# BosonHBC/BHRayTracer

Hardware: AMD Instinct MI355X
Metric: Mrays/s (closest-hit + any-hit rays per second), with wall-clock per frame (higher is better)
Workload: dtype f32

## Files before the change

### bhraytracer_amd/__init__.py

```python
import ctypes as C
import os

import numpy as np

from .flat import FlatView

_HERE = os.path.dirname(os.path.abspath(__file__))
LIB_PATH = os.environ.get("BHRT_LIB") or os.path.join(_HERE, "libbhrt.so")

SIDE_FRONT, SIDE_BACK, SIDE_BOTH = 1, 2, 3


class BhrtError(RuntimeError):
    pass


class Info(C.Structure):
    _fields_ = [("width", C.c_int32), ("height", C.c_int32)] + [
        (n, C.c_uint32) for n in ("n_nodes", "n_meshes", "n_triangles", "n_bvh_nodes", "n_materials", "n_lights",
                                  "n_textures", "max_node_depth", "max_bvh_depth")] + [
        ("flat_bytes", C.c_uint64), ("n_warnings", C.c_uint32)]


class Opts(C.Structure):
    _fields_ = [("spp", C.c_int32), ("gi_bounces", C.c_int32), ("internal_bounces", C.c_int32), ("seed", C.c_uint32),
                ("jitter", C.c_int32), ("gamma", C.c_int32), ("photon_map", C.c_int32),
                ("rank", C.c_int32), ("world_size", C.c_int32), ("tile_size", C.c_int32),
                ("samples_per_pass", C.c_int32), ("timers", C.c_int32), ("photon_exact", C.c_int32), ("leaf_skip", C.c_int32), ("photon_radius", C.c_float), ("lens", C.c_int32)]


class Stats(C.Structure):
    _fields_ = [("closest_rays", C.c_uint64), ("shadow_rays", C.c_uint64), ("shade_calls", C.c_uint64),
                ("camera_samples", C.c_uint64), ("passes", C.c_uint32), ("wave_iterations", C.c_uint32),
                ("seconds_total", C.c_double), ("seconds_trace_closest", C.c_double),
                ("seconds_trace_shadow", C.c_double), ("seconds_shade", C.c_double), ("seconds_other", C.c_double),
                ("launches_trace_closest", C.c_uint64), ("launches_trace_shadow", C.c_uint64),
                ("seconds_photon_gather", C.c_double), ("seconds_photon_heavy", C.c_double),
                ("photon_queries", C.c_uint64), ("photon_heavy_queries", C.c_uint64), ("photon_wave_queries", C.c_uint64),
                ("photon_exact_queries", C.c_uint64), ("photon_nodes_visited", C.c_uint64), ("deferred_rays", C.c_uint64),
                ("photon_lane_queries", C.c_uint64), ("photon_lane_nodes", C.c_uint64), ("photon_found", C.c_uint64), ("reserved", C.c_double * 1)]

    def as_dict(self):
        return {n: getattr(self, n) for n, _ in self._fields_ if n != "reserved"}


class DenoiseOpts(C.Structure):
    _fields_ = [("iterations", C.c_int32), ("sigma_normal", C.c_float), ("sigma_depth", C.c_float), ("sigma_luminance", C.c_float),
                ("gamma", C.c_int32), ("reserved", C.c_int32 * 3)]


class AdaptiveOpts(C.Structure):
    _fields_ = [("min_spp", C.c_int32), ("threshold", C.c_float), ("floor", C.c_float), ("reserved", C.c_int32 * 5)]


class Hits(C.Structure):
    _fields_ = [("t", C.c_void_p), ("node", C.c_void_p), ("prim", C.c_void_p), ("front", C.c_void_p)]


_lib = None

EXPORTS = [
    "bhrt_last_error", "bhrt_default_opts", "bhrt_scene_load_xml", "bhrt_scene_free", "bhrt_scene_info",
    "bhrt_scene_warning", "bhrt_scene_flat", "bhrt_scene_upload", "bhrt_device_count",
# ... 362 lines not shown
```

### bhraytracer_amd/csrc/device_color24.h

```cpp
#pragma once
#include <stddef.h>
#include <stdint.h>

#include "bhrt_detmath.h"
#include "vecmath.h"

namespace bhrt {

__device__ inline void store_color24(uint8_t *rgb8, size_t pix, V3 out, int gamma)
{
    if (gamma) {
        const float inv = 1 / 2.2f;
        out = v3(dm::powf_(out.x, inv), dm::powf_(out.y, inv), dm::powf_(out.z, inv));
    }
    int r = int(out.x * 255 + 0.5f), g = int(out.y * 255 + 0.5f), b = int(out.z * 255 + 0.5f);
    rgb8[pix * 3] = (uint8_t)(r < 0 ? 0 : (r > 255 ? 255 : r));
    rgb8[pix * 3 + 1] = (uint8_t)(g < 0 ? 0 : (g > 255 ? 255 : g));
    rgb8[pix * 3 + 2] = (uint8_t)(b < 0 ? 0 : (b > 255 ? 255 : b));
}

}
```

### bhraytracer_amd/csrc/device_state.h

```cpp
#pragma once

namespace bhrt {

template <class T> struct DevBuf {
    T *p = nullptr;
    size_t n = 0;
    DevBuf() = default;
    DevBuf(const DevBuf &) = delete;
    DevBuf &operator=(const DevBuf &) = delete;
    DevBuf(DevBuf &&o) noexcept : p(o.p), n(o.n) { o.p = nullptr; o.n = 0; }
    DevBuf &operator=(DevBuf &&o) noexcept
    {
        if (this != &o) { Free(); p = o.p; n = o.n; o.p = nullptr; o.n = 0; }
        return *this;
    }
    ~DevBuf() { Free(); }
    int Reserve(size_t want)
    {
        if (n >= want) return BHRT_OK;
        Free();
        HIP_CHECK(hipMalloc(&p, want * sizeof(T)));
        n = want;
        return BHRT_OK;
    }
// ... 49 lines not shown
        if (stream2) (void)hipStreamDestroy(stream2);
        if (stream) (void)hipStreamDestroy(stream);
    }
};

struct DeviceState : DeviceQueues {
    int device = -1;
    uint32_t n_cus = 256;
    DevBuf<uint8_t> d_blob;
    DevBuf<int32_t> d_chain;
    DevBuf<float> d_aux;
    DevScene S;
    uint32_t cap_samples = 0, cap_rays = 0, cap_frames = 0;
    DevBuf<float> d_rayf[2];
    DevBuf<uint32_t> d_rayu[2];
    DevBuf<float> d_hitf;
    DevBuf<int32_t> d_hiti;
    DevBuf<float> d_shf;
    DevBuf<uint32_t> d_shu;
    DevBuf<uint32_t> d_fu;
    DevBuf<uint64_t> d_fcode;
    DevBuf<float> d_ff;
    DevBuf<float> d_samples;
    DevBuf<uint32_t> d_order;
    uint32_t order_shard_cap = 0;
    DevBuf<uint32_t> d_seg;
    DevBuf<uint32_t> d_park;
    DevBuf<float> d_slowf;
    DevBuf<uint32_t> d_slowu;
    DevBuf<float> d_shf2;
    DevBuf<uint32_t> d_shu2;
    DevBuf<uint32_t> d_order_sh;
    DevBuf<uint32_t> d_seg_sh;
    DevBuf<Counters> d_cnt_sh;
    DevBuf<Counters> d_cnt;
    PinnedBuf<HostCounters> h_pub;
    HostCounters *d_pub = nullptr;
    uint32_t pub_seq = 0;
    int timers = 0;
    int photon_exact = 0;
    uint32_t *d_knn = nullptr;
    DevBuf<uint32_t> d_sel;
    struct PendingTimer { int e0, e1; double *acc; };
    std::vector<PendingTimer> ev_pending;
    std::vector<int> ev_free;
    DevBuf<DPhoton> d_photons;
// ... 3 lines not shown
    DevBuf<float4> d_ph_hot, d_ph_cold, d_ph_dbox;
    PhotonMapDev pm;
    DevBuf<unsigned long long> d_scr;
    uint32_t scr_lanes = 0;
    uint32_t heavy_cap = 0;
    DevBuf<uint32_t> d_heavy;
    DevBuf<uint32_t> d_long;
    DevBuf<uint32_t> d_cell_of, d_gorder, d_rank_of, d_keys_out;
    DevBuf<uint8_t> d_sort_temp;
    size_t sort_temp_bytes = 0;
    DevBuf<uint32_t> d_n_heavy;
    PinnedBuf<uint32_t> h_n_heavy;
    DevBuf<uint32_t> d_cells, d_tile_sums;
    struct Knobs {
        int stream_waves = -1;
        bool fused_camera = true;
        bool no_slow_queue = false;
        bool debug_slow = false, debug_gather = false, debug_drain = false;
        bool balance_host = false;
        int frame_cap = 0;
        int gather_lane_budget = 0;
        bool gather_counting_sort = false;
        bool shadow_overlap = true;
        int gather_stats = 0;
        void FromEnv()
        {
            if (const char *e = getenv("BHRT_STREAM_WAVES")) stream_waves = atoi(e);
            if (const char *e = getenv("BHRT_FUSED_CAMERA")) fused_camera = atoi(e) != 0;
            no_slow_queue = getenv("BHRT_NO_SLOW_QUEUE") != nullptr;
            debug_slow = getenv("BHRT_DEBUG_SLOW") != nullptr; debug_gather = getenv("BHRT_DEBUG_GATHER") != nullptr; debug_drain = getenv("BHRT_DEBUG_DRAIN") != nullptr;
            if (const char *e = getenv("BHRT_PHOTON_BALANCE_HOST")) balance_host = atoi(e) != 0;
            if (const char *e = getenv("BHRT_GATHER_COUNTING_SORT")) gather_counting_sort = atoi(e) != 0;
            if (const char *e = getenv("BHRT_SHADOW_OVERLAP")) shadow_overlap = atoi(e) != 0;
        }
    } knobs;
    uint64_t pass_hint_key = 0;
    uint32_t pass_hint = 0;
    uint64_t frames_seen_key = 0;
    double frames_seen = 0;
    size_t frame_px = 0;
    DevBuf<uint8_t> d_frame_rgb;
    DevBuf<float> d_frame_rad, d_frame_var;
    DevBuf<uint32_t> d_frame_cnt;
    DevBuf<uint8_t> d_ad;
    DevBuf<uint8_t> d_dn;
    size_t api_cap = 0;
    DevBuf<float> d_api_f;
    DevBuf<int32_t> d_api_i;
};

void DestroyDeviceState(DeviceState *d)
{
    if (!d) return;
    if (d->device >= 0) (void)hipSetDevice(d->device);
    delete d;
}
// ... 3 lines not shown
```

### bhraytracer_amd/csrc/kernels.hip

```cpp
#include <hip/hip_runtime.h>

#include <stdlib.h>
#include <string.h>

#include <algorithm>
#include <type_traits>
#include <chrono>
#include <string>
#include <vector>

#include "bhrt.h"
#include "denoise.h"
#include "device_color24.h"
#include "device_photon.h"
#include "photon_host.h"
#include "scene_internal.h"

namespace bhrt {

#define HIP_CHECK(expr)                                                                                        \
    do {                                                                                                       \
        hipError_t e_ = (expr);                                                                                \
        if (e_ != hipSuccess) {                                                                                \
            SetError(std::string(#expr) + ": " + hipGetErrorString(e_));                                       \
// ... 100 lines not shown
    __syncthreads();
    if (threadIdx.x < 3) {
        const uint32_t k = threadIdx.x;
        uint32_t sum = 0;
        for (int w = 0; w < kShadeWaves; w++) { const uint32_t t = L.total[k][w]; L.base[k][w] = sum; sum += t; }
        uint32_t *ctr = k == 0 ? c0 : (k == 1 ? c1 : c2);
        const uint32_t b = (sum && ctr) ? atomicAdd(ctr, sum) : 0u;
        for (int w = 0; w < kShadeWaves; w++) L.base[k][w] += b;
    }
    __syncthreads();
    s0a = L.base[0][wave] + pa;
    s0b = L.base[0][wave] + ta + pb;
    s1 = L.base[1][wave] + (uint32_t)__popcll(m1 & lt);
    s2 = L.base[2][wave] + (uint32_t)__popcll(m2 & lt);
    __syncthreads();
}

__device__ inline uint32_t sample_addr(const PassInfo &P, uint32_t slot)
{
    uint32_t px, smp;
    fdivmod(slot, P.by_spp, px, smp);
    return smp * P.n_pixels + px;
}

__device__ inline void put_ray(const RayQueue &q, uint32_t i, V3 o, V3 d, uint32_t frame, uint32_t meta, uint32_t ctr)
{
    q.ox[i] = o.x; q.oy[i] = o.y; q.oz[i] = o.z; q.dx[i] = d.x; q.dy[i] = d.y; q.dz[i] = d.z;
    q.frame[i] = frame; q.meta[i] = meta;
    if ((meta & 15u) != RK_GI) q.rng_ctr[i] = ctr;
}
__device__ inline uint32_t make_meta(uint32_t kind, uint32_t side, int bounce) { return kind | (side << 4) | ((uint32_t)(bounce & 0xff) << 8); }
__device__ inline void st3(float *a, uint32_t i, V3 v) { a[3 * (size_t)i] = v.x; a[3 * (size_t)i + 1] = v.y; a[3 * (size_t)i + 2] = v.z; }
__device__ inline V3 ld3i(const float *a, uint32_t i) { return v3(a[3 * (size_t)i], a[3 * (size_t)i + 1], a[3 * (size_t)i + 2]); }

template <bool kLens = false>
__device__ inline bool camera_ray(const DevScene &S, const PassInfo &P, uint32_t idx, V3 &o, V3 &d)
{
    int i = 0, j = 0;
    uint32_t s;
    o = v3(0, 0, 0); d = v3(0, 0, 0);
    if (!slot_pixel(P, idx, i, j, s)) return false;
    const V3 topLeft = ld3(S.cam.top_left), ddx = ld3(S.cam.dd_x), ddy = ld3(S.cam.dd_y), pos = ld3(S.cam.pos);
    V3 target = (topLeft + (float)i * ddx) - (float)j * ddy;
    if (P.jitter) {
        const float pixelLen = P.pixel_len;
        const V3 ux = ld3(P.jx), uy = ld3(P.jy);
// ... 606 lines not shown
                    out.has_shadow = true;
                    out.so = a.p;
                    out.sd = light.size > 0 ? sample_along_normal(g, centerDir, light.size) : centerDir;
                    out.stmax = 1;
                }
            }
            const V3 kd = kd_s, ks = ks_s;
            st3(F.brdf, f, kd * cosTheta + ks * dm::powf_(dot(vH, vN), m.glossiness));
        }
    }
    if (R.photon) {
        st3(F.ph_p, f, a.p); st3(F.ph_n, f, a.N); st3(F.ph_v, f, vV);
        st3(F.ph_kd, f, kd_s);
        st3(F.ph_ks, f, ks_s);
    }
    F.info[f] = how | (dmode << 3) | (light_idx << 8) | (flags << 16) | ((uint32_t)(mi & 0xfff) << 20);
}

#ifndef BHRT_SHADE_WAVES
#define BHRT_SHADE_WAVES 4
#endif
template <bool kCamera, bool kTex, bool kFused = false>
__device__ __forceinline__ void shade_block(const DevScene &S, const RenderParams &R, const PassInfo &P, const RayQueue &qin, const HitBuf &hb, uint32_t n, const RayQueue &qout,
                                            const ShadowQueue &qs, const Frames &F, float *samples, Counters *cnt, const RayOrder &ord)
{
    static_assert(!kFused || kCamera, "only camera rays are traced in the shading kernel");
    __shared__ BlockAllocLds lds;
    uint32_t seg = 0, local = 0, i;
    bool active;
    if (kFused) {
        i = blockIdx.x * kShadeBlock + threadIdx.x;
        active = i < n;
        if (!active) i = 0;
    } else {
        constexpr uint32_t kSegs = 3 * BHRT_ORDER_SHARDS;
        __shared__ uint32_t s_seg;
        if (threadIdx.x < 64) {
            const uint32_t l = threadIdx.x;
            const uint32_t a = ord.seg_start[l], b = (l + 64 < kSegs) ? ord.seg_start[l + 64] : 0xffffffffu;
            const uint32_t n_le = (uint32_t)__popcll(__ballot(a <= blockIdx.x)) + (uint32_t)__popcll(__ballot(b <= blockIdx.x));
            if (l == 0) s_seg = n_le - 1;
        }
        __syncthreads();
        seg = s_seg;
        if (blockIdx.x >= ord.seg_start[kSegs]) return;
        const uint32_t seg_cnt = ord.seg_count[seg];
        const uint32_t bb = blockIdx.x - ord.seg_start[seg];
// ... 28 lines not shown
    uint32_t f, u2;
    if (kFused) { uint32_t u0, u1; block_alloc3(lds, &cnt->n_frames.v, new_frame ? 1u : 0u, 0u, nullptr, 0u, nullptr, 0u, f, u0, u1, u2); }
    else f = ord.frame_base[seg] + local;
    if (new_frame && f >= R.cap_frames) { flag_overflow(cnt, 1u); new_frame = false; }

    ShadeOut so;
    so.has_refr = so.has_gi = so.has_shadow = false;
    uint32_t ray_owner = owner;

    if (new_frame) {
        uint64_t code = 1;
        uint32_t skey;
        int gi;
        uint32_t how;
        V3 mult = v3(1, 1, 1);
        if (kind == RK_CAMERA) {
            int pi, pj;
            uint32_t osmp;
            slot_pixel(P, owner, pi, pj, osmp);
            skey = bhrt_sample_key(P.seed, (uint32_t)(pj * P.W + pi), P.s0 + osmp);
            gi = R.gi_bounces;
            bounce = R.internal_bounces;
            how = FH_ROOT;
        } else {
            const uint64_t pcode = F.code[owner];
            skey = F.skey[owner];
            const uint32_t pi2 = F.info2[owner];
            gi = (int)(pi2 & 0xffu) - 64 - 1;
            if (kind == RK_GI) {
                code = pcode * 2 + 1;
                how = FH_GI;
                bounce = (int)((pi2 >> 8) & 0xffu);
            } else if (kind == RK_REFR_IN) {
                code = pcode * 2;
                how = FH_REFR_FRONT;
            } else {
                code = pcode * 2;
                how = FH_REFR_OUT;
                const bhrt_material &pm = S.materials[(F.info[owner] >> 20) & 0xfffu];
                V3 af = v3(dm::powf_(BHRT_EULER, -pm.absorption[0] * hit.t), dm::powf_(BHRT_EULER, -pm.absorption[1] * hit.t),
                           dm::powf_(BHRT_EULER, -pm.absorption[2] * hit.t));
                mult = ld3i(F.refr_color, owner) * af;
            }
        }
        F.parent[f] = owner;
        F.info2[f] = (uint32_t)(gi + 64) | ((uint32_t)(bounce & 0xff) << 8);
        F.skey[f] = skey;
        F.code[f] = code;
        if (how == FH_REFR_OUT) st3(F.mult, f, mult);
        const int mi = S.nodes[hit.node].material;
        const bool need_uv = kTex && mi >= 0 && (S.materials[mi].diffuse.map >= 0 || S.materials[mi].specular.map >= 0);
        Attr a;
        hit_attrs(S, o, d, hit.t, hit.node, hit.prim, need_uv, a);
        shade_entry<kTex>(S, R, F, f, how, o, a, hit.node, bounce, gi, code, skey, so);
        ray_owner = f;
    } else if (active) {
        if (kind == RK_CAMERA) {
            int pi, pj;
            uint32_t osmp;
            slot_pixel(P, owner, pi, pj, osmp);
            st3(samples, sample_addr(P, owner), kTex ? tc_sample(S, S.background, v3((float)pi / S.cam.width, (float)pj / S.cam.height, 0.0f)) : ld3(S.background.color));
        } else if (kind == RK_GI) {
            V3 mult = ld3i(F.gi_mult, owner);
            V3 outc = v3(0, 0, 0);
            if (is_hit) {
                outc = outc + v3(0, 0, 0) * mult;
            } else if (d.x == d.y && d.x == 0) {
                outc = outc + v3(1.0f, 0.0f, 1.0f);
            } else {
                V3 env = (kTex ? sample_environment(S, S.environment, d) : ld3(S.environment.color)) * mult;
                if (!(isnan_f(env.x) || isnan_f(env.y) || isnan_f(env.z))) outc = outc + env;
            }
            if (isnan_f(outc.x)) outc = v3(1.0f, 0.0f, 1.0f);
            else outc = clamp_white(outc);
            st3(F.gi, owner, outc);
        } else if (kind == RK_REFR_IN) {
            if (!is_hit) {
                st3(F.refr, owner, v3(1.0f, 0.0f, 1.0f));
            } else {
                Attr a;
                hit_attrs(S, o, d, hit.t, hit.node, hit.prim, false, a);
                const bhrt_material &m = S.materials[(F.info[owner] >> 20) & 0xfffu];
                const float refrGloss = m.glossiness > 50 ? m.glossiness : 0.f;
                V3 vN = a.N;
// ... 41 lines not shown
            st3(F.refr, owner, clamp_white(ld3i(F.refr_color, owner) * (kTex ? sample_environment(S, S.environment, d) : ld3(S.environment.color))));
        }
    }

    uint32_t r0, r1, s0;
    block_alloc3(lds, &cnt->n_next.v, so.has_refr ? 1u : 0u, so.has_gi ? 1u : 0u, &cnt->n_shadow.v, so.has_shadow ? 1u : 0u, nullptr, 0u, r0, r1, s0, u2);
    if (so.has_refr) {
        if (r0 < R.cap_rays) put_ray(qout, r0, so.ro, so.rd, ray_owner, so.rmeta, so.rctr);
        else flag_overflow(cnt, 2u);
    }
    if (so.has_gi) {
        if (r1 < R.cap_rays) put_ray(qout, r1, so.go, so.gd, ray_owner, make_meta(RK_GI, BHRT_HIT_FRONT, 0), 0);
        else flag_overflow(cnt, 2u);
    }
    if (so.has_shadow) {
        if (s0 < R.cap_shadow) {
            qs.ox[s0] = so.so.x; qs.oy[s0] = so.so.y; qs.oz[s0] = so.so.z; qs.dx[s0] = so.sd.x; qs.dy[s0] = so.sd.y; qs.dz[s0] = so.sd.z;
            qs.tmax[s0] = so.stmax; qs.frame[s0] = ray_owner;
        } else flag_overflow(cnt, 4u);
    }
}
template <bool kCamera, bool kTex, bool kFused = false>
__global__ void __launch_bounds__(kShadeBlock, BHRT_SHADE_WAVES) k_shade(DevScene S, RenderParams R, PassInfo P, RayQueue qin, HitBuf hb, uint32_t n, RayQueue qout,
                                                   ShadowQueue qs, Frames F, float *samples, Counters *cnt, RayOrder ord, HostCounters *pub, uint32_t seq)
{
    shade_block<kCamera, kTex, kFused>(S, R, P, qin, hb, n, qout, qs, F, samples, cnt, ord);
    if (!pub) return;
    __syncthreads();
    if (threadIdx.x == 0 && atomicAdd(&cnt->shade_done.v, 1u) == gridDim.x - 1u) {
        __hip_atomic_store(&cnt->shade_done.v, 0u, __ATOMIC_RELAXED, __HIP_MEMORY_SCOPE_AGENT);
        publish_counters(cnt, pub, seq);
    }
}

__global__ void __launch_bounds__(kBlock) k_combine(DevScene S, PassInfo P, Frames F, uint32_t f0, uint32_t f1, float *samples, int photon)
{
    const uint32_t f = f0 + blockIdx.x * blockDim.x + threadIdx.x;
    if (f >= f1) return;
    const uint32_t info = F.info[f];
    const uint32_t how = info & 7u, dmode = (info >> 3) & 7u, li = (info >> 8) & 0xffu, flags = (info >> 16) & 0xfu;
    V3 out;
    if (flags & FF_CONST) out = ld3i(F.refr, f);
    else {
        out = v3(0, 0, 0);
        if (flags & FF_HAS_REFR) out = out + ld3i(F.refr, f);
        bool done = out.x >= 1 && out.y >= 1 && out.z >= 1;
        if (!done) {
            if (flags & FF_HAS_GI) out = out + ld3i(F.gi, f);
            done = out.x >= 1 && out.y >= 1 && out.z >= 1;
        }
        if (!done) {
            V3 dc = v3(0, 0, 0);
            if (dmode != DM_NONE) {
                const bhrt_light &l = S.lights[li];
                V3 I = ld3(l.intensity), irrad;
                const float vis = F.vis[f];
                if (dmode == DM_AMBIENT) irrad = I;
                else if (dmode == DM_DIRECT) irrad = vis * I;
                else if (dmode == DM_POINT) irrad = (vis * I) / F.rr[f];
                else irrad = v3(1, 1, 1) * BHRT_BIGFLOAT;
                dc = dc + irrad * ld3i(F.brdf, f);
            }
            if (photon) dc = dc + ld3i(F.caustic, f);
            dc = clamp_white(dc);
            if (isnan_f(dc.x)) dc = v3(0, 0, 0);
            out = out + dc;
            done = out.x >= 1 && out.y >= 1 && out.z >= 1;
            if (!done && isnan_f(out.x)) out = v3(1.0f, 0.0f, 1.0f);
        }
    }
    const uint32_t parent = F.parent[f];
    if (how == FH_ROOT) st3(samples, sample_addr(P, parent), out);
    else if (how == FH_GI) {
        V3 oc = v3(0, 0, 0) + out * ld3i(F.gi_mult, parent);
        if (isnan_f(oc.x)) oc = v3(1.0f, 0.0f, 1.0f);
        else oc = clamp_white(oc);
        st3(F.gi, parent, oc);
    } else if (how == FH_REFR_FRONT) st3(F.refr, parent, clamp_white(out));
    else st3(F.refr, parent, clamp_white(ld3i(F.mult, f) * out));
}

__global__ void __launch_bounds__(kBlock) k_resolve(PassInfo P, const float *samples, float *radiance, uint8_t *rgb8)
{
    const uint32_t q = blockIdx.x * blockDim.x + threadIdx.x;
    if (q >= P.n_pixels) return;
    int i, j;
    if (!pixel_of(P, pass_pixel(P, q), i, j)) return;
    V3 sum = v3(0, 0, 0);
    for (int s = 0; s < P.spp; s++) sum = sum + ld3i(samples, (uint32_t)s * P.n_pixels + q);
    V3 out = sum / (float)P.spp;
    const size_t pix = (size_t)j * P.W + i;
    if (radiance) st3(radiance, (uint32_t)pix, out);
    if (rgb8) store_color24(rgb8, pix, out, P.gamma);
}

__global__ void __launch_bounds__(kBlock) k_variance(PassInfo P, const float *samples, float *variance)
{
    const uint32_t q = blockIdx.x * blockDim.x + threadIdx.x;
    if (q >= P.n_pixels) return;
    int i, j;
    if (!pixel_of(P, pass_pixel(P, q), i, j)) return;
    V3 sum = v3(0, 0, 0);
    for (int s = 0; s < P.spp; s++) sum = sum + ld3i(samples, (uint32_t)s * P.n_pixels + q);
    const V3 m = sum / (float)P.spp;
    V3 acc = v3(0, 0, 0);
    if (P.spp > 1) {
        for (int s = 0; s < P.spp; s++) {
            const V3 d = ld3i(samples, (uint32_t)s * P.n_pixels + q) - m;
            acc = acc + d * d;
        }
        acc = (acc / (float)(P.spp - 1)) / (float)P.spp;
    }
    st3(variance, (uint32_t)((size_t)j * P.W + i), acc);
}

struct AdaptState {
// ... 578 lines not shown
}

static int EnsureUploaded(bhrt_scene *scene)
{
    if (!scene) { SetError("null scene"); return BHRT_ERR_ARG; }
    if (scene->dev) { HIP_CHECK(hipSetDevice(scene->dev->device)); return BHRT_OK; }
    return bhrt_scene_upload(scene, 0);
}

static int EnsureWorkspace(DeviceState *D, uint32_t cap_samples, double frames_per_sample)
{
    const size_t cf_wanted = (size_t)std::ceil((double)cap_samples * frames_per_sample);
    if (cf_wanted > 0xffffffffull) { SetError("frame pool beyond 2^32 frames"); return BHRT_ERR_ARG; }
    if (D->cap_samples >= cap_samples && D->cap_frames >= cf_wanted) return BHRT_OK;
    const size_t cr = (size_t)cap_samples * 2, cf = cf_wanted;
    const uint32_t shard_cap = (uint32_t)(2 * ((((cr + 1023) / 1024 + BHRT_ORDER_SHARDS - 1) / BHRT_ORDER_SHARDS) * 1024 + 1024));
    auto each = [&](auto f) -> int {
        int rc = BHRT_OK;
        auto go = [&](auto &buf, size_t n) { if (!rc) rc = f(buf, n); };
        for (int k = 0; k < 2; k++) { go(D->d_rayf[k], cr * 6); go(D->d_rayu[k], cr * 3); }
        go(D->d_hitf, cr); go(D->d_hiti, cr * 3); go(D->d_shf, cr * 7); go(D->d_shu, cr);
        go(D->d_fu, cf * 4); go(D->d_fcode, cf); go(D->d_ff, cf * 23);
        go(D->d_samples, (size_t)cap_samples * 3);
        go(D->d_order, (size_t)4 * BHRT_ORDER_SHARDS * shard_cap);
        go(D->d_park, 3 * cr + (1u << BHRT_PARK_KEY_BITS) + kScanBlock);
        if (D->stream3) { go(D->d_shf2, cr * 7); go(D->d_shu2, cr); go(D->d_order_sh, (size_t)BHRT_ORDER_SHARDS * shard_cap); }
        return rc;
    };
    each([](auto &buf, size_t) { buf.Free(); return BHRT_OK; });
    D->cap_samples = 0;
    BHRT_TRY(each([](auto &buf, size_t n) { return buf.Reserve(n); }));
    D->order_shard_cap = shard_cap;
    D->cap_samples = cap_samples; D->cap_rays = (uint32_t)cr; D->cap_frames = (uint32_t)cf;
    D->d_ph_frames.Free();
    return BHRT_OK;
}

static uint32_t DefaultPassSamples(DeviceState *D, bool photon_map, double frames_per_sample)
{
    const double frame_b = 116 + (photon_map ? 60 : 0);
    const double per_sample = 2 * (72 + 16 + 32 + 40 + (D->stream3 ? 32 + 8 : 0)) + 12 + frames_per_sample * frame_b;
    size_t free_b = 0, total_b = 0;
    if (hipMemGetInfo(&free_b, &total_b) != hipSuccess) return 1u << 26;
    const double have = (double)D->cap_samples * (2 * (72 + 16 + 32 + 40 + (D->stream3 ? 32 + 8 : 0)) + 12) + (double)D->cap_frames * frame_b;
    for (uint32_t p = 1u << 28; p > (1u << 22); p >>= 1)
        if ((D->cap_samples >= p && (double)D->cap_frames >= (double)p * frames_per_sample) || (double)p * per_sample <= 0.85 * ((double)free_b + have)) return p;
    return 1u << 22;
}

static Frames MakeFrames(DeviceState *D)
{
    Frames F;
    const size_t c = D->cap_frames;
    F.parent = D->d_fu; F.info = D->d_fu + c; F.info2 = D->d_fu + 2 * c; F.skey = D->d_fu + 3 * c;
// ... 264 lines not shown
        V.RO_sh.mesh_start = D->d_seg_sh; V.RO_sh.mesh_count = D->d_seg_sh + BHRT_ORDER_SHARDS + 1;
    }
    V.slowq.q = MakeRayQueue(D->d_slowf, D->d_slowu, kSlowCap);
    V.slowq.cap = D->d_slowf && !D->knobs.no_slow_queue ? kSlowCap : 0u;
    V.slow_hits = MakeHitBuf(D->d_slowf ? D->d_slowf + (size_t)6 * kSlowCap : nullptr, (int32_t *)(D->d_slowu ? D->d_slowu + (size_t)3 * kSlowCap : nullptr), kSlowCap);
    return V;
}

static void LaunchAnyHit(DeviceState *D, hipStream_t stream, bool meshes, const ShadowQueue &sq, uint32_t n, const uint32_t *n_dev, float *vis, const RayOrder &order,
                         Counters *counters, int path_mode, bool ls, double *seconds)
{
    Timer t(D, seconds, 1, stream);
    const dim3 hg((n + kBlock - 1) / kBlock), hb(kBlock);
    if (meshes) {
        hipLaunchKernelGGL(k_trace_shadow_park, hg, hb, 0, stream, D->S, sq, n, n_dev, vis, order, counters);
        hipLaunchKernelGGL(k_mesh_prefix, dim3(1), dim3(64), 0, stream, counters, order);
        hipLaunchKernelGGL(path_mode == 1 ? (ls ? k_shadow_mesh<1, true> : k_shadow_mesh<1>) : path_mode == 2 ? (ls ? k_shadow_mesh<2, true> : k_shadow_mesh<2>) : k_shadow_mesh<0>, dim3((hg.x + BHRT_ORDER_SHARDS) * (kBlock / kShadowBlock)), dim3(kShadowBlock), 0, stream, D->S, sq, vis, order);
    } else hipLaunchKernelGGL(k_trace_shadow<false>, hg, hb, 0, stream, D->S, sq, n, n_dev, vis);
    t.Stop();
}

template <class Consume>
static int RenderPixels(bhrt_scene *scene, const bhrt_opts &o, PassInfo P, const uint32_t *d_list, uint64_t n_items, uint32_t s0, uint32_t spp, bhrt_stats *st,
                        const Consume &consume)
{
    DeviceState *D = scene->dev;
    const bhrt_flat_header *H = scene->flat.hdr();
    const int tile = P.tile, world = P.world;
    P.spp = (int32_t)spp; P.by_spp = MakeFastDiv(spp); P.s0 = s0;

    const uint64_t frames_key = RenderKey(o, spp, world, tile);
    double frames_per_sample = 6.0;
    bool frames_learned = false;
    if (o.samples_per_pass <= 0 && D->frames_seen_key == frames_key && D->frames_seen > 0 && D->frames_seen < 4.0 &&
        n_items * (uint64_t)spp > DefaultPassSamples(D, o.photon_map != 0, 6.0)) {
        frames_per_sample = std::min(6.0, D->frames_seen * 1.3 + 0.25);
        frames_learned = true;
    }
    uint32_t pass_samples = o.samples_per_pass > 0 ? (uint32_t)o.samples_per_pass : DefaultPassSamples(D, o.photon_map != 0, frames_per_sample);
    pass_samples = (uint32_t)std::min<uint64_t>(pass_samples, std::max<uint64_t>(n_items * (uint64_t)spp, 1));
    if (pass_samples < spp) pass_samples = spp;
    D->timers = o.timers;
    D->photon_exact = o.photon_exact;
    const bool ls = o.leaf_skip != 0;
    int path_mode = 1;
    {
        const bhrt_mesh *hm = (const bhrt_mesh *)(scene->flat.blob.data() + H->off_meshes);
// ... 9 lines not shown

    uint64_t q = 0;
    uint32_t pass_limit = 0;
    const uint64_t hint_key = frames_key ^ ((uint64_t)pass_samples << 1);
    if (D->pass_hint_key == hint_key && D->pass_hint) pass_limit = D->pass_hint;
    while (q < n_items) {
        int rc = EnsureWorkspace(D, pass_samples, frames_per_sample);
        if (rc) return rc;
        R.cap_rays = D->cap_rays; R.cap_shadow = D->cap_rays; R.cap_frames = D->cap_frames;
        if (D->knobs.frame_cap > 0) R.cap_frames = std::min<uint32_t>(R.cap_frames, (uint32_t)D->knobs.frame_cap);
        if (o.photon_map) BHRT_TRY(D->d_ph_frames.Reserve((size_t)D->cap_frames * 15));
        if (pass_limit == 0) pass_limit = pass_samples;
        if (pass_limit > D->cap_samples) pass_limit = D->cap_samples;
        const uint32_t px_per_pass = pass_limit / spp;
        const uint32_t npx = (uint32_t)std::min<uint64_t>(px_per_pass, n_items - q);
        if (d_list) { P.list = d_list + q; P.q0 = 0; } else P.q0 = (uint32_t)q;
        P.n_pixels = npx;
        const bool sh_overlap = D->knobs.shadow_overlap && D->stream3 != nullptr && D->d_shf2.p != nullptr;
        const PassViews V = MakePassViews(D, sh_overlap);
        const Frames &F = V.F;
        const RayOrder &RO = V.RO;
        bool sh_pending[2] = {false, false};
        HIP_CHECK(hipMemsetAsync(D->d_cnt, 0, sizeof(Counters), D->stream));
        const uint32_t total = npx * spp;
        uint32_t n_cur = total;
        bool first_step = true;
        const bool lens = P.lens_r > 0.f;
        if (lens) {
            Timer t(D, &st->seconds_other);
            hipLaunchKernelGGL(k_lens_rays, dim3((total + kBlock - 1) / kBlock), dim3(kBlock), 0, D->stream, D->S, P, V.Q[0], total);
            t.Stop();
        }
        int cur = 0;
        std::vector<uint32_t> frame_marks = {0};
        bool overflow = false;
        uint64_t pass_closest = 0, pass_camera = 0, pass_shadow = 0, pass_deferred = 0;
        uint32_t pass_steps = 0;
        const SlowQueue no_slow = {V.slowq.q, 0u};
        uint32_t slow_pending = 0, slow_traced = 0, slow_injected = 0;
        struct SlowBatch { uint32_t end; uint32_t step; hipEvent_t done; };
        std::vector<SlowBatch> slow_batches;
        size_t slow_batch_next = 0;
#ifndef BHRT_INJECT_MIN_LOG2
#define BHRT_INJECT_MIN_LOG2 20
#endif
        constexpr uint32_t kInjectMinRays = 1u << BHRT_INJECT_MIN_LOG2;
// ... 90 lines not shown
                    else
                    hipLaunchKernelGGL(mesh_kernel, cam_step ? dim3(tg.x + BHRT_ORDER_SHARDS)  : dim3((n_cur + kMeshBlock - 1) / kMeshBlock),
                                       cam_step ? tb : dim3(kMeshBlock), 0, D->stream, D->S, P, V.Q[cur], V.HB, RO, D->d_cnt);
                    if (!cam_step) hipLaunchKernelGGL(k_file_parked, dim3(tg.x + BHRT_ORDER_SHARDS), tb, 0, D->stream, V.Q[cur], V.HB, RO, D->d_cnt);
                } else if (cam_step) hipLaunchKernelGGL(HIP_KERNEL_NAME(k_trace_closest<false, true, false>), tg, tb, 0, D->stream, D->S, P, V.Q[cur], n_cur, 0, V.HB, RO, D->d_cnt, no_slow);
                else hipLaunchKernelGGL(HIP_KERNEL_NAME(k_trace_closest<false, false, false>), tg, tb, 0, D->stream, D->S, P, V.Q[cur], n_cur, 0, V.HB, RO, D->d_cnt, no_slow);
                t.Stop();
            }
            if (n_extra) hipLaunchKernelGGL(k_file_all, dim3(kFileAllBlocks(n_cur, n_cur + n_extra)), dim3(kBlock), 0, D->stream, V.Q[cur], V.HB, n_cur, n_cur + n_extra, RO, D->d_cnt);
            if (!fused) {
                st->launches_trace_closest++;
                hipLaunchKernelGGL(k_order_prefix, dim3(1), dim3(128), 0, D->stream, D->d_cnt, RO);
            }
            const uint32_t seq = ++D->pub_seq;
            {
                Timer t(D, &st->seconds_shade, 0);
                const dim3 sg((n_cur + n_extra + kShadeBlock - 1) / kShadeBlock + (fused ? 0 : 3 * BHRT_ORDER_SHARDS)), sb(kShadeBlock);
                const bool tex = H->n_texmaps > 0;
                auto shade = fused ? (tex ? k_shade<true, true, true> : k_shade<true, false, true>)
                                   : cam_step ? (tex ? k_shade<true, true> : k_shade<true, false>) : (tex ? k_shade<false, true> : k_shade<false, false>);
                const int par = (int)(pass_steps & 1u);
                if (sh_wait_n) { HIP_CHECK(hipEventRecord(D->ev_shade, D->stream)); rc = launch_any_hit(D->ev_shade); if (rc) return rc; }
                if (sh_overlap && sh_pending[par]) { HIP_CHECK(hipStreamWaitEvent(D->stream, D->ev_shadow[par], 0)); sh_pending[par] = false; }
                hipLaunchKernelGGL(shade, sg, sb, 0, D->stream, D->S, R, P, V.Q[cur], V.HB, n_cur + n_extra, V.Q[cur ^ 1], (sh_overlap && par) ? V.SQ2 : V.SQ, F, D->d_samples, D->d_cnt, RO, D->d_pub, seq);
                t.Stop();
                if (sh_overlap) HIP_CHECK(hipEventRecord(D->ev_shade, D->stream));
            }
            if (!sh_overlap) {
                LaunchAnyHit(D, D->stream, H->n_meshes > 0, V.SQ, std::min<uint32_t>(n_cur + n_extra, R.cap_shadow), &D->d_cnt->n_shadow.v, F.vis, RO, D->d_cnt, path_mode, ls,
                             &st->seconds_trace_shadow);
            }
            rc = WaitPublished(D, seq);
            if (rc) return rc;
            const HostCounters hc = *D->h_pub;
            FlushTimers(D);
            if (hc.overflow) { overflow = true; break; }
            if (first_step) {
                const uint64_t valid_px = d_list ? npx : CountValidPixels(P, npx);
                pass_closest = valid_px * (uint64_t)spp;
                pass_camera = pass_closest;
                first_step = false;
            } else if (!injected) pass_closest += n_cur;
            slow_pending = std::min<uint32_t>(hc.n_slow, kSlowCap);
            if (slow_pending > slow_traced) {
                const uint32_t cnt_new = slow_pending - slow_traced;
                hipLaunchKernelGGL(k_trace_slow, dim3(cnt_new), dim3(64), 0, D->stream2, D->S, V.slowq, slow_traced, slow_pending, V.slow_hits);
                if (D->knobs.debug_slow) fprintf(stderr, "slow rays: %u set aside in wave step %u at %.1f ms\n", cnt_new, pass_steps, std::chrono::duration<double>(std::chrono::steady_clock::now() - wall0).count() * 1e3);
// ... 34 lines not shown
                    w[0], w[0] ? (double)w[1] / w[0] : 0., w[2], w[2] ? (double)w[3] / w[2] : 0., w[4], w[4] ? (double)w[5] / w[4] : 0., w[6], w[6] ? (double)w[7] / w[6] : 0., w[8],
                    w[8] ? (double)w[9] / w[8] : 0., w[10], w[10] ? (double)w[11] / w[10] : 0., w[12], w[13], w[14], w[15]);
            fprintf(stderr, "stream: %llu rounds (%llu descend, %llu leaf), walking %.3f, in phase %.3f, clocks in rounds %.3g of which descend rounds %.3g, %llu refills\n", d[0], d[6],
                    d[7], d[0] ? (double)d[1] / (64.0 * d[0]) : 0.0, d[0] ? (double)d[2] / (64.0 * d[0]) : 0.0, (double)d[3], (double)d[4], d[5]);
        }
#endif
        st->camera_samples += pass_camera; st->shadow_rays += pass_shadow; st->wave_iterations += pass_steps; st->deferred_rays += pass_deferred;
        {
            const double seen = (double)frame_marks.back() / (double)std::max<uint64_t>((uint64_t)npx * (uint64_t)spp, 1);
            if (D->frames_seen_key != frames_key) { D->frames_seen_key = frames_key; D->frames_seen = 0; }
            D->frames_seen = std::max(D->frames_seen, seen);
        }
        if (o.photon_map && frame_marks.back() > 0) {
            Timer t(D, &st->seconds_photon_gather, 0);
            const GatherToFrames sink = {F, D->S.materials};
            int rc = RunGather(D, sink, 0, frame_marks.back(), o.photon_radius > 0.f ? o.photon_radius : 0.5f , st);
            if (rc) return rc;
            t.Stop();
        }
        st->shade_calls += D->h_pub->n_frames;
        st->closest_rays += pass_closest;
        {
            Timer t(D, &st->seconds_other);
            for (size_t k = frame_marks.size(); k-- > 1;) {
                const uint32_t f0 = frame_marks[k - 1], f1 = frame_marks[k];
                if (f1 > f0) hipLaunchKernelGGL(k_combine, dim3((f1 - f0 + kBlock - 1) / kBlock), dim3(kBlock), 0, D->stream, D->S, P, F, f0, f1, D->d_samples, o.photon_map);
            }
            consume(P, npx);
            t.Stop();
        }
        HIP_CHECK(hipGetLastError());
        st->passes++;
        q += npx;
    }
    return BHRT_OK;
}

static int RenderRange(bhrt_scene *scene, const bhrt_opts &o, uint8_t *d_rgb8, float *d_radiance, bhrt_stats *st, float *d_region_samples, int x0,
                       int y0, int x1, int y1, float *d_variance = nullptr)
{
    DeviceState *D = scene->dev;
    PassInfo P;
    uint64_t owned_pixels = 0;
    int rc = FramePassInfo(scene, o, P, owned_pixels);
    if (rc) return rc;
    const auto wall0 = std::chrono::steady_clock::now();
    rc = RenderPixels(scene, o, P, nullptr, owned_pixels, 0, (uint32_t)o.spp, st, [&](const PassInfo &Pp, uint32_t npx) {
        hipLaunchKernelGGL(k_resolve, dim3((npx + kBlock - 1) / kBlock), dim3(kBlock), 0, D->stream, Pp, D->d_samples, d_radiance, d_rgb8);
        if (d_variance) hipLaunchKernelGGL(k_variance, dim3((npx + kBlock - 1) / kBlock), dim3(kBlock), 0, D->stream, Pp, D->d_samples, d_variance);
        if (d_region_samples)
            hipLaunchKernelGGL(k_copy_samples, dim3((npx + kBlock - 1) / kBlock), dim3(kBlock), 0, D->stream, Pp, D->d_samples, x0, y0, x1, y1, d_region_samples);
    });
    if (rc) return rc;
    HIP_CHECK(hipStreamSynchronize(D->stream));
    FlushTimers(D, true);
    st->seconds_total += std::chrono::duration<double>(std::chrono::steady_clock::now() - wall0).count();
    return BHRT_OK;
}

static int RenderAdaptive(bhrt_scene *scene, const bhrt_opts &o, const bhrt_adaptive_opts &ao, uint8_t *d_rgb8, float *d_radiance, float *d_variance,
                          uint32_t *d_count, bhrt_stats *st)
{
    DeviceState *D = scene->dev;
    PassInfo P;
    uint64_t owned_pixels = 0;
    int rc = FramePassInfo(scene, o, P, owned_pixels);
    if (rc) return rc;
    if (owned_pixels > 0xffffffffull) { SetError("adaptive render: more than 2^32 owned pixels"); return BHRT_ERR_ARG; }
    BHRT_TRY(D->d_ad.Reserve((size_t)owned_pixels * 44 + 16));
    const size_t N = (D->d_ad.n - 16) / 44;
    AdaptState A;
    A.a = (float4 *)D->d_ad.p; A.b = A.a + N; A.c = (float *)(A.b + N);
    uint32_t *lists[2] = {(uint32_t *)(A.c + N), (uint32_t *)(A.c + N) + N};
    AdaptParams R;
    R.n_max = (uint32_t)o.spp; R.threshold = ao.threshold; R.floor = ao.floor;
    R.radiance = d_radiance; R.variance = d_variance; R.rgb8 = d_rgb8; R.count = d_count;
    R.n_next = lists[1] + N;
    const auto wall0 = std::chrono::steady_clock::now();
    uint32_t n_prev = 0, n = (uint32_t)ao.min_spp;
    uint64_t items = owned_pixels;
    const uint32_t *list = nullptr;
    for (int cur = 0; items > 0; cur ^= 1) {
        R.next = lists[cur];
        HIP_CHECK(hipMemsetAsync(R.n_next, 0, sizeof(uint32_t), D->stream));
        rc = RenderPixels(scene, o, P, list, items, n_prev, n - n_prev, st, [&](const PassInfo &Pp, uint32_t npx) {
            hipLaunchKernelGGL(k_adapt_fold, dim3((npx + kBlock - 1) / kBlock), dim3(kBlock), 0, D->stream, Pp, D->d_samples, A, R);
        });
        if (rc) return rc;
        uint32_t active = 0;
        HIP_CHECK(hipMemcpyAsync(&active, R.n_next, sizeof active, hipMemcpyDeviceToHost, D->stream));
        HIP_CHECK(hipStreamSynchronize(D->stream));
        if (n >= (uint32_t)o.spp && active) { SetError("adaptive render: pixels active after the last round"); return BHRT_ERR_HIP; }
        items = active;
        list = lists[cur];
        n_prev = n;
        n = (uint32_t)std::min<uint64_t>((uint64_t)o.spp, 2ull * n);
    }
    HIP_CHECK(hipStreamSynchronize(D->stream));
    FlushTimers(D, true);
    st->seconds_total += std::chrono::duration<double>(std::chrono::steady_clock::now() - wall0).count();
    return BHRT_OK;
}

static const char *LensArgsError(const bhrt_scene *scene, const bhrt_opts *o)
{
    if (!scene || !o) return "";
    if (o->lens != 0 && o->lens != 1) return "lens must be 0 (pinhole) or 1 (thin lens)";
    const float dof = scene->flat.hdr()->camera.dof;
// ... 61 lines not shown
using namespace bhrt;

extern "C" {

int bhrt_device_count(int *n)
try {
    if (!n) { SetError("null argument"); return BHRT_ERR_ARG; }
    int c = 0;
    hipError_t e = hipGetDeviceCount(&c);
    if (e != hipSuccess) { *n = 0; SetError(std::string("hipGetDeviceCount: ") + hipGetErrorString(e)); return BHRT_ERR_NO_DEVICE; }
    *n = c;
    return BHRT_OK;
} catch (...) { return bhrt::AbiException(); }

int bhrt_scene_knob(bhrt_scene *scene, const char *name, int value)
try {
    int rc = EnsureUploaded(scene);
    if (rc) return rc;
    if (!name || value < 0) { SetError("knob: bad arguments"); return BHRT_ERR_ARG; }
    if (!strcmp(name, "frame_cap")) scene->dev->knobs.frame_cap = value;
    else if (!strcmp(name, "gather_lane_budget")) scene->dev->knobs.gather_lane_budget = value;
    else if (!strcmp(name, "gather_stats")) scene->dev->knobs.gather_stats = value;
    else if (!strcmp(name, "shadow_overlap")) scene->dev->knobs.shadow_overlap = value != 0;
    else { SetError(std::string("knob: unknown name ") + name); return BHRT_ERR_ARG; }
    return BHRT_OK;
} catch (...) { return bhrt::AbiException(); }

int bhrt_scene_upload(bhrt_scene *scene, int device)
try {
    if (!scene) { SetError("null scene"); return BHRT_ERR_ARG; }
    if (scene->dev && scene->dev->device == device) { HIP_CHECK(hipSetDevice(device)); return BHRT_OK; }
    int count = 0;
    if (hipGetDeviceCount(&count) != hipSuccess || count <= 0) { SetError("no HIP device available (this path has no CPU fallback)"); return BHRT_ERR_NO_DEVICE; }
    if (device < 0 || device >= count) { SetError("device index out of range"); return BHRT_ERR_ARG; }
    if (scene->max_bvh_depth > 64) { SetError("BVH deeper than 64 levels: the stackless trail holds 64"); return BHRT_ERR_UNSUPPORTED; }
    if (scene->dev) { DestroyDeviceState(scene->dev); scene->dev = nullptr; }
    HIP_CHECK(hipSetDevice(device));
    DeviceState *D = new DeviceState;
    D->knobs.FromEnv();
    D->device = device;
    scene->dev = D;
    {
        int cus = 0;
        if (hipDeviceGetAttribute(&cus, hipDeviceAttributeMultiprocessorCount, device) == hipSuccess && cus > 0) D->n_cus = (uint32_t)cus;
    }
    const std::vector<uint8_t> &blob = scene->flat.blob;
// ... 895 lines not shown
```

### include/bhrt.h

```cpp
#ifndef BHRT_H
#define BHRT_H
#include <stddef.h>
#include <stdint.h>

#ifdef __cplusplus
extern "C" {
#endif

typedef struct bhrt_scene bhrt_scene;

#define BHRT_SIDE_FRONT 1
#define BHRT_SIDE_BACK 2
#define BHRT_SIDE_BOTH 3

enum {
    BHRT_OK = 0,
    BHRT_ERR_IO = 1,
    BHRT_ERR_PARSE = 2,
    BHRT_ERR_ARG = 3,
    BHRT_ERR_NO_DEVICE = 4,
    BHRT_ERR_HIP = 5,
    BHRT_ERR_UNSUPPORTED = 6,
    BHRT_ERR_OVERFLOW = 7
};
// ... 22 lines not shown
    int32_t leaf_skip;
    float photon_radius;
    int32_t lens;
} bhrt_opts;

typedef struct bhrt_stats {
    uint64_t closest_rays;
    uint64_t shadow_rays;
    uint64_t shade_calls;
    uint64_t camera_samples;
    uint32_t passes, wave_iterations;
    double seconds_total;
    double seconds_trace_closest, seconds_trace_shadow, seconds_shade, seconds_other;
    uint64_t launches_trace_closest, launches_trace_shadow;
    double seconds_photon_gather;
    double seconds_photon_heavy;
    uint64_t photon_queries;
    uint64_t photon_heavy_queries;
    uint64_t photon_wave_queries;
    uint64_t photon_exact_queries;
    uint64_t photon_nodes_visited;
    uint64_t deferred_rays;
    uint64_t photon_lane_queries, photon_lane_nodes, photon_found;
    double reserved[1];
} bhrt_stats;

typedef struct bhrt_hits {
    float *t;
    int32_t *node;
    int32_t *prim;
    int32_t *front;
} bhrt_hits;

const char *bhrt_last_error(void);
void bhrt_default_opts(bhrt_opts *opts);

int bhrt_scene_load_xml(const char *path, bhrt_scene **out);
int bhrt_scene_load_xml_ex(const char *path, int bvh_device, bhrt_scene **out);
struct bhrt_bvh_node;
int bhrt_bvh_build(const float *vertices, uint32_t n_vertices, const uint32_t *faces, uint32_t n_faces, uint32_t max_per_leaf, int device,
                   struct bhrt_bvh_node *nodes_out, uint32_t node_capacity, uint32_t *n_nodes, uint32_t *elems_out, uint32_t *depth);
int bhrt_scene_clone(const bhrt_scene *scene, bhrt_scene **out);
void bhrt_scene_free(bhrt_scene *scene);
int bhrt_scene_info(const bhrt_scene *scene, bhrt_info *info);
int bhrt_scene_warning(const bhrt_scene *scene, uint32_t i, const char **text);
int bhrt_scene_flat(const bhrt_scene *scene, const void **blob, uint64_t *bytes);
int bhrt_scene_set_lens(bhrt_scene *scene, float focaldist, float dof);
// ... 81 lines not shown
```

Before: 6612.

## Fuse root-frame combine with pixel resolve via per-sample root frame index

Camera shading records each sample's root frame index (or a sentinel for background) instead of writing the sample buffer. A new resolve kernel evaluates root frame values directly and averages them per pixel in shared memory, writing radiance and RGB8. This skips the last k_combine launch and the samples round trip for plain renders. It adds a root index buffer and a more complex resolve kernel with per-block shared-memory reductions, and it only applies when variance and region outputs are not requested.

```diff
diff --git a/bhraytracer_amd/__init__.py b/bhraytracer_amd/__init__.py
--- a/bhraytracer_amd/__init__.py
+++ b/bhraytracer_amd/__init__.py
@@ -38,7 +38,7 @@
                 ("seconds_photon_gather", C.c_double), ("seconds_photon_heavy", C.c_double),
                 ("photon_queries", C.c_uint64), ("photon_heavy_queries", C.c_uint64), ("photon_wave_queries", C.c_uint64),
                 ("photon_exact_queries", C.c_uint64), ("photon_nodes_visited", C.c_uint64), ("deferred_rays", C.c_uint64),
-                ("photon_lane_queries", C.c_uint64), ("photon_lane_nodes", C.c_uint64), ("photon_found", C.c_uint64), ("reserved", C.c_double * 1)]
+                ("photon_lane_queries", C.c_uint64), ("photon_lane_nodes", C.c_uint64), ("photon_found", C.c_uint64), ("launches_resolve_fused", C.c_uint64)]
 
     def as_dict(self):
         return {n: getattr(self, n) for n, _ in self._fields_ if n != "reserved"}
diff --git a/bhraytracer_amd/csrc/device_color24.h b/bhraytracer_amd/csrc/device_color24.h
--- a/bhraytracer_amd/csrc/device_color24.h
+++ b/bhraytracer_amd/csrc/device_color24.h
@@ -7,16 +7,17 @@
 
 namespace bhrt {
 
+__device__ inline uint8_t color24_channel(float v, int gamma)
+{
+    if (gamma) v = dm::powf_(v, 1 / 2.2f);
+    const int b = int(v * 255 + 0.5f);
+    return (uint8_t)(b < 0 ? 0 : (b > 255 ? 255 : b));
+}
 __device__ inline void store_color24(uint8_t *rgb8, size_t pix, V3 out, int gamma)
 {
-    if (gamma) {
-        const float inv = 1 / 2.2f;
-        out = v3(dm::powf_(out.x, inv), dm::powf_(out.y, inv), dm::powf_(out.z, inv));
-    }
-    int r = int(out.x * 255 + 0.5f), g = int(out.y * 255 + 0.5f), b = int(out.z * 255 + 0.5f);
-    rgb8[pix * 3] = (uint8_t)(r < 0 ? 0 : (r > 255 ? 255 : r));
-    rgb8[pix * 3 + 1] = (uint8_t)(g < 0 ? 0 : (g > 255 ? 255 : g));
-    rgb8[pix * 3 + 2] = (uint8_t)(b < 0 ? 0 : (b > 255 ? 255 : b));
+    rgb8[pix * 3] = color24_channel(out.x, gamma);
+    rgb8[pix * 3 + 1] = color24_channel(out.y, gamma);
+    rgb8[pix * 3 + 2] = color24_channel(out.z, gamma);
 }
 
 }
diff --git a/bhraytracer_amd/csrc/device_state.h b/bhraytracer_amd/csrc/device_state.h
--- a/bhraytracer_amd/csrc/device_state.h
+++ b/bhraytracer_amd/csrc/device_state.h
@@ -95,6 +95,7 @@
     DevBuf<uint64_t> d_fcode;
     DevBuf<float> d_ff;
     DevBuf<float> d_samples;
+    DevBuf<uint32_t> d_root;
     DevBuf<uint32_t> d_order;
     uint32_t order_shard_cap = 0;
     DevBuf<uint32_t> d_seg;
@@ -144,6 +145,7 @@
         int gather_lane_budget = 0;
         bool gather_counting_sort = false;
         bool shadow_overlap = true;
+        bool fused_resolve = true;
         int gather_stats = 0;
         void FromEnv()
         {
@@ -154,6 +156,7 @@
             if (const char *e = getenv("BHRT_PHOTON_BALANCE_HOST")) balance_host = atoi(e) != 0;
             if (const char *e = getenv("BHRT_GATHER_COUNTING_SORT")) gather_counting_sort = atoi(e) != 0;
             if (const char *e = getenv("BHRT_SHADOW_OVERLAP")) shadow_overlap = atoi(e) != 0;
+            if (const char *e = getenv("BHRT_FUSED_RESOLVE")) fused_resolve = atoi(e) != 0;
         }
     } knobs;
     uint64_t pass_hint_key = 0;
diff --git a/bhraytracer_amd/csrc/kernels.hip b/bhraytracer_amd/csrc/kernels.hip
--- a/bhraytracer_amd/csrc/kernels.hip
+++ b/bhraytracer_amd/csrc/kernels.hip
@@ -146,6 +146,7 @@
     fdivmod(slot, P.by_spp, px, smp);
     return smp * P.n_pixels + px;
 }
+constexpr uint32_t kNoRootFrame = 0xffffffffu;
 
 __device__ inline void put_ray(const RayQueue &q, uint32_t i, V3 o, V3 d, uint32_t frame, uint32_t meta, uint32_t ctr)
 {
@@ -798,7 +799,7 @@
 #endif
 template <bool kCamera, bool kTex, bool kFused = false>
 __device__ __forceinline__ void shade_block(const DevScene &S, const RenderParams &R, const PassInfo &P, const RayQueue &qin, const HitBuf &hb, uint32_t n, const RayQueue &qout,
-                                            const ShadowQueue &qs, const Frames &F, float *samples, Counters *cnt, const RayOrder &ord)
+                                            const ShadowQueue &qs, const Frames &F, float *samples, uint32_t *root_of, Counters *cnt, const RayOrder &ord)
 {
     static_assert(!kFused || kCamera, "only camera rays are traced in the shading kernel");
     __shared__ BlockAllocLds lds;
@@ -873,6 +874,7 @@
             gi = R.gi_bounces;
             bounce = R.internal_bounces;
             how = FH_ROOT;
+            if (root_of) root_of[owner] = f;
         } else {
             const uint64_t pcode = F.code[owner];
             skey = F.skey[owner];
@@ -909,8 +911,11 @@
         if (kind == RK_CAMERA) {
             int pi, pj;
             uint32_t osmp;
-            slot_pixel(P, owner, pi, pj, osmp);
-            st3(samples, sample_addr(P, owner), kTex ? tc_sample(S, S.background, v3((float)pi / S.cam.width, (float)pj / S.cam.height, 0.0f)) : ld3(S.background.color));
+            if (root_of) root_of[owner] = kNoRootFrame;
+            else {
+                slot_pixel(P, owner, pi, pj, osmp);
+                st3(samples, sample_addr(P, owner), kTex ? tc_sample(S, S.background, v3((float)pi / S.cam.width, (float)pj / S.cam.height, 0.0f)) : ld3(S.background.color));
+            }
         } else if (kind == RK_GI) {
             V3 mult = ld3i(F.gi_mult, owner);
             V3 outc = v3(0, 0, 0);
@@ -998,9 +1003,9 @@
 }
 template <bool kCamera, bool kTex, bool kFused = false>
 __global__ void __launch_bounds__(kShadeBlock, BHRT_SHADE_WAVES) k_shade(DevScene S, RenderParams R, PassInfo P, RayQueue qin, HitBuf hb, uint32_t n, RayQueue qout,
-                                                   ShadowQueue qs, Frames F, float *samples, Counters *cnt, RayOrder ord, HostCounters *pub, uint32_t seq)
-{
-    shade_block<kCamera, kTex, kFused>(S, R, P, qin, hb, n, qout, qs, F, samples, cnt, ord);
+                                                   ShadowQueue qs, Frames F, float *samples, uint32_t *root_of, Counters *cnt, RayOrder ord, HostCounters *pub, uint32_t seq)
+{
+    shade_block<kCamera, kTex, kFused>(S, R, P, qin, hb, n, qout, qs, F, samples, root_of, cnt, ord);
     if (!pub) return;
     __syncthreads();
     if (threadIdx.x == 0 && atomicAdd(&cnt->shade_done.v, 1u) == gridDim.x - 1u) {
@@ -1009,12 +1014,9 @@
     }
 }
 
-__global__ void __launch_bounds__(kBlock) k_combine(DevScene S, PassInfo P, Frames F, uint32_t f0, uint32_t f1, float *samples, int photon)
-{
-    const uint32_t f = f0 + blockIdx.x * blockDim.x + threadIdx.x;
-    if (f >= f1) return;
-    const uint32_t info = F.info[f];
-    const uint32_t how = info & 7u, dmode = (info >> 3) & 7u, li = (info >> 8) & 0xffu, flags = (info >> 16) & 0xfu;
+__device__ inline V3 frame_value(const DevScene &S, const Frames &F, uint32_t f, uint32_t info, int photon)
+{
+    const uint32_t dmode = (info >> 3) & 7u, li = (info >> 8) & 0xffu, flags = (info >> 16) & 0xfu;
     V3 out;
     if (flags & FF_CONST) out = ld3i(F.refr, f);
     else {
@@ -1045,6 +1047,16 @@
             if (!done && isnan_f(out.x)) out = v3(1.0f, 0.0f, 1.0f);
         }
     }
+    return out;
+}
+
+__global__ void __launch_bounds__(kBlock) k_combine(DevScene S, PassInfo P, Frames F, uint32_t f0, uint32_t f1, float *samples, int photon)
+{
+    const uint32_t f = f0 + blockIdx.x * blockDim.x + threadIdx.x;
+    if (f >= f1) return;
+    const uint32_t info = F.info[f];
+    const uint32_t how = info & 7u;
+    const V3 out = frame_value(S, F, f, info, photon);
     const uint32_t parent = F.parent[f];
     if (how == FH_ROOT) st3(samples, sample_addr(P, parent), out);
     else if (how == FH_GI) {
@@ -1068,6 +1080,56 @@
     const size_t pix = (size_t)j * P.W + i;
     if (radiance) st3(radiance, (uint32_t)pix, out);
     if (rgb8) store_color24(rgb8, pix, out, P.gamma);
+}
+
+constexpr int kResolvePixels = 8;
+constexpr int kResolveStride = 64 * 3 + 3;
+template <bool kTex>
+__global__ void __launch_bounds__(64) k_resolve_frames(DevScene S, PassInfo P, Frames F, const uint32_t *root_of, int photon, float *radiance, uint8_t *rgb8)
+{
+    __shared__ float s_val[kResolvePixels * kResolveStride];
+    const uint32_t lane = threadIdx.x, spp = (uint32_t)P.spp;
+    const uint32_t q0 = blockIdx.x * kResolvePixels;
+    const uint32_t n_here = min((uint32_t)kResolvePixels, P.n_pixels - q0);
+    const uint32_t sp = lane / 3u, sc = lane - 3u * sp;
+    int si = 0, sj = 0;
+    const bool summing = sp < n_here && pixel_of(P, pass_pixel(P, q0 + sp), si, sj);
+    float sum = 0.f;
+    for (uint32_t s0 = 0; s0 < spp; s0 += 64u) {
+        const uint32_t smp = s0 + lane;
+        uint32_t f[kResolvePixels], info[kResolvePixels];
+        bool live[kResolvePixels];
+        int pi[kResolvePixels], pj[kResolvePixels];
+#pragma unroll
+        for (int p = 0; p < kResolvePixels; p++) {
+            pi[p] = pj[p] = 0;
+            live[p] = (uint32_t)p < n_here && pixel_of(P, pass_pixel(P, q0 + p), pi[p], pj[p]) && smp < spp;
+            f[p] = live[p] ? root_of[(q0 + p) * spp + smp] : kNoRootFrame;
+        }
+#pragma unroll
+        for (int p = 0; p < kResolvePixels; p++) info[p] = f[p] != kNoRootFrame ? F.info[f[p]] : 0u;
+#pragma unroll
+        for (int p = 0; p < kResolvePixels; p++) {
+            if (!live[p]) continue;
+            V3 v;
+            if (f[p] != kNoRootFrame) v = frame_value(S, F, f[p], info[p], photon);
+            else v = kTex ? tc_sample(S, S.background, v3((float)pi[p] / S.cam.width, (float)pj[p] / S.cam.height, 0.0f)) : ld3(S.background.color);
+            float *dst = s_val + p * kResolveStride + 3 * lane;
+            dst[0] = v.x; dst[1] = v.y; dst[2] = v.z;
+        }
+        __syncthreads();
+        if (summing) {
+            const float *src = s_val + sp * kResolveStride + sc;
+            const uint32_t n = min(64u, spp - s0);
+            for (uint32_t s = 0; s < n; s++) sum = sum + src[3 * s];
+        }
+        __syncthreads();
+    }
+    if (!summing) return;
+    const float m = sum / (float)P.spp;
+    const size_t pix = (size_t)sj * P.W + si;
+    if (radiance) radiance[pix * 3 + sc] = m;
+    if (rgb8) rgb8[pix * 3 + sc] = color24_channel(m, P.gamma);
 }
 
 __global__ void __launch_bounds__(kBlock) k_variance(PassInfo P, const float *samples, float *variance)
@@ -1692,6 +1754,7 @@
         go(D->d_hitf, cr); go(D->d_hiti, cr * 3); go(D->d_shf, cr * 7); go(D->d_shu, cr);
         go(D->d_fu, cf * 4); go(D->d_fcode, cf); go(D->d_ff, cf * 23);
         go(D->d_samples, (size_t)cap_samples * 3);
+        go(D->d_root, cap_samples);
         go(D->d_order, (size_t)4 * BHRT_ORDER_SHARDS * shard_cap);
         go(D->d_park, 3 * cr + (1u << BHRT_PARK_KEY_BITS) + kScanBlock);
         if (D->stream3) { go(D->d_shf2, cr * 7); go(D->d_shu2, cr); go(D->d_order_sh, (size_t)BHRT_ORDER_SHARDS * shard_cap); }
@@ -1700,6 +1763,7 @@
     each([](auto &buf, size_t) { buf.Free(); return BHRT_OK; });
     D->cap_samples = 0;
     BHRT_TRY(each([](auto &buf, size_t n) { return buf.Reserve(n); }));
+    HIP_CHECK(hipMemset(D->d_root, 0xff, (size_t)cap_samples * sizeof(uint32_t)));
     D->order_shard_cap = shard_cap;
     D->cap_samples = cap_samples; D->cap_rays = (uint32_t)cr; D->cap_frames = (uint32_t)cf;
     D->d_ph_frames.Free();
@@ -2010,7 +2074,7 @@
 
 template <class Consume>
 static int RenderPixels(bhrt_scene *scene, const bhrt_opts &o, PassInfo P, const uint32_t *d_list, uint64_t n_items, uint32_t s0, uint32_t spp, bhrt_stats *st,
-                        const Consume &consume)
+                        bool fuse_root, const Consume &consume)
 {
     DeviceState *D = scene->dev;
     const bhrt_flat_header *H = scene->flat.hdr();
@@ -2066,6 +2130,7 @@
         const RayOrder &RO = V.RO;
         bool sh_pending[2] = {false, false};
         HIP_CHECK(hipMemsetAsync(D->d_cnt, 0, sizeof(Counters), D->stream));
+        uint32_t *const root_of = fuse_root ? D->d_root.p : nullptr;
         const uint32_t total = npx * spp;
         uint32_t n_cur = total;
         bool first_step = true;
@@ -2202,7 +2267,7 @@
                 const int par = (int)(pass_steps & 1u);
                 if (sh_wait_n) { HIP_CHECK(hipEventRecord(D->ev_shade, D->stream)); rc = launch_any_hit(D->ev_shade); if (rc) return rc; }
                 if (sh_overlap && sh_pending[par]) { HIP_CHECK(hipStreamWaitEvent(D->stream, D->ev_shadow[par], 0)); sh_pending[par] = false; }
-                hipLaunchKernelGGL(shade, sg, sb, 0, D->stream, D->S, R, P, V.Q[cur], V.HB, n_cur + n_extra, V.Q[cur ^ 1], (sh_overlap && par) ? V.SQ2 : V.SQ, F, D->d_samples, D->d_cnt, RO, D->d_pub, seq);
+                hipLaunchKernelGGL(shade, sg, sb, 0, D->stream, D->S, R, P, V.Q[cur], V.HB, n_cur + n_extra, V.Q[cur ^ 1], (sh_overlap && par) ? V.SQ2 : V.SQ, F, D->d_samples, root_of, D->d_cnt, RO, D->d_pub, seq);
                 t.Stop();
                 if (sh_overlap) HIP_CHECK(hipEventRecord(D->ev_shade, D->stream));
             }
@@ -2283,11 +2348,11 @@
         st->closest_rays += pass_closest;
         {
             Timer t(D, &st->seconds_other);
-            for (size_t k = frame_marks.size(); k-- > 1;) {
+            for (size_t k = frame_marks.size(); k-- > (fuse_root ? 2 : 1);) {
                 const uint32_t f0 = frame_marks[k - 1], f1 = frame_marks[k];
                 if (f1 > f0) hipLaunchKernelGGL(k_combine, dim3((f1 - f0 + kBlock - 1) / kBlock), dim3(kBlock), 0, D->stream, D->S, P, F, f0, f1, D->d_samples, o.photon_map);
             }
-            consume(P, npx);
+            consume(P, npx, F);
             t.Stop();
         }
         HIP_CHECK(hipGetLastError());
@@ -2306,7 +2371,15 @@
     int rc = FramePassInfo(scene, o, P, owned_pixels);
     if (rc) return rc;
     const auto wall0 = std::chrono::steady_clock::now();
-    rc = RenderPixels(scene, o, P, nullptr, owned_pixels, 0, (uint32_t)o.spp, st, [&](const PassInfo &Pp, uint32_t npx) {
+    const bool fuse_root = D->knobs.fused_resolve && !d_variance && !d_region_samples;
+    const bool tex = scene->flat.hdr()->n_texmaps > 0;
+    rc = RenderPixels(scene, o, P, nullptr, owned_pixels, 0, (uint32_t)o.spp, st, fuse_root, [&](const PassInfo &Pp, uint32_t npx, const Frames &F) {
+        if (fuse_root) {
+            hipLaunchKernelGGL(tex ? k_resolve_frames<true> : k_resolve_frames<false>, dim3((npx + kResolvePixels - 1) / kResolvePixels), dim3(64), 0, D->stream, D->S, Pp, F,
+                               D->d_root.p, o.photon_map, d_radiance, d_rgb8);
+            st->launches_resolve_fused++;
+            return;
+        }
         hipLaunchKernelGGL(k_resolve, dim3((npx + kBlock - 1) / kBlock), dim3(kBlock), 0, D->stream, Pp, D->d_samples, d_radiance, d_rgb8);
         if (d_variance) hipLaunchKernelGGL(k_variance, dim3((npx + kBlock - 1) / kBlock), dim3(kBlock), 0, D->stream, Pp, D->d_samples, d_variance);
         if (d_region_samples)
@@ -2344,7 +2417,7 @@
     for (int cur = 0; items > 0; cur ^= 1) {
         R.next = lists[cur];
         HIP_CHECK(hipMemsetAsync(R.n_next, 0, sizeof(uint32_t), D->stream));
-        rc = RenderPixels(scene, o, P, list, items, n_prev, n - n_prev, st, [&](const PassInfo &Pp, uint32_t npx) {
+        rc = RenderPixels(scene, o, P, list, items, n_prev, n - n_prev, st, false, [&](const PassInfo &Pp, uint32_t npx, const Frames &) {
             hipLaunchKernelGGL(k_adapt_fold, dim3((npx + kBlock - 1) / kBlock), dim3(kBlock), 0, D->stream, Pp, D->d_samples, A, R);
         });
         if (rc) return rc;
@@ -2452,6 +2525,7 @@
     else if (!strcmp(name, "gather_lane_budget")) scene->dev->knobs.gather_lane_budget = value;
     else if (!strcmp(name, "gather_stats")) scene->dev->knobs.gather_stats = value;
     else if (!strcmp(name, "shadow_overlap")) scene->dev->knobs.shadow_overlap = value != 0;
+    else if (!strcmp(name, "fused_resolve")) scene->dev->knobs.fused_resolve = value != 0;
     else { SetError(std::string("knob: unknown name ") + name); return BHRT_ERR_ARG; }
     return BHRT_OK;
 } catch (...) { return bhrt::AbiException(); }
diff --git a/include/bhrt.h b/include/bhrt.h
--- a/include/bhrt.h
+++ b/include/bhrt.h
@@ -68,7 +68,7 @@
     uint64_t photon_nodes_visited;
     uint64_t deferred_rays;
     uint64_t photon_lane_queries, photon_lane_nodes, photon_found;
-    double reserved[1];
+    uint64_t launches_resolve_fused;
 } bhrt_stats;
 
 typedef struct bhrt_hits {
```

Result: faster. 6747, median of 6 (+2.0%).
